# aleju/cat-generator

Measured on AMD Instinct MI355X. Metric: images/sec per G+D step, G32up-c 32x32 RGB bs=128 per GPU, higher is better.
Workload: dtype f32

## Files before the change

cat-generator_amd/csrc/common.h:

```cpp
#pragma once
#include <hip/hip_runtime.h>
#include <algorithm>
#include <stdint.h>
#include <stdio.h>
#include <string.h>
#include "../../include/catgan.h"

namespace cg {

char* err_buf();
int fail(const char* fmt, ...);

inline hipStream_t S(void* s) { return reinterpret_cast<hipStream_t>(s); }

#define CG_HIP(call)                                                              \
    do {                                                                          \
        hipError_t e__ = (call);                                                  \
        if (e__ != hipSuccess)                                                    \
            return cg::fail("%s:%d %s -> %s", __FILE__, __LINE__, #call,          \
                            hipGetErrorString(e__));                              \
    } while (0)

#define CG_LAUNCH_CHECK()                                                         \
    do {                                                                          \
        hipError_t e__ = hipGetLastError();                                       \
        if (e__ != hipSuccess)                                                    \
            return cg::fail("%s:%d kernel launch -> %s", __FILE__, __LINE__,      \
                            hipGetErrorString(e__));                              \
    } while (0)

#define CG_REQUIRE(cond, ...)                                                     \
    do {                                                                          \
        if (!(cond)) return cg::fail(__VA_ARGS__);                                \
    } while (0)

constexpr int kNumCU = 256;

#ifndef CG_TIMING_PROBE
#define CG_TIMING_PROBE 0
#endif
#define CG_PROBE_HALF(fam, T) (((CG_TIMING_PROBE) & (fam)) ? ((T) + 1) / 2 : (T))
constexpr int kEwWgsPerCU = 4, kColReduceWgsPerCU = 1;

enum Opt {
    OPT_SKINNY, OPT_GEMM_BK32, OPT_WINO_BK, OPT_NN_TILE, OPT_TN_TILE, OPT_NN_SPLITS, OPT_TN_SPLITS,
    OPT_XCD_SWIZZLE, OPT_NN_GLDS, OPT_TN_GLDS, OPT_WINO_GLDS, OPT_PAD_SKIP, OPT_WINO3, OPT_WINO_DGRAD_FUSE, OPT_WINO_DGRAD_FUSE_LAUNCHES,
    OPT_COUNT
};
long opt(Opt o);
void opt_count(Opt o);

static inline int cdiv(long a, long b) { return (int)((a + b - 1) / b); }

constexpr size_t kColScratchBytes = 8u << 20;
void* col_scratch(hipStream_t stream);
hipStream_t queue_stream(hipStream_t ref, int cls, int slot);
int queue_class(hipStream_t ref, hipStream_t s);
void wgrad_discard_all();

constexpr int kSkinnyWgradBlocks = 512;
bool skinny_ok(int ngroups, int Cin, int Cout, int kH, int kW, int padH, int padW, int ups);
size_t skinny_wgrad_ws_bytes(int Cin, int Cout);
void skinny_valu_forward(hipStream_t st, const float* x, const float* w, const float* bias, float* y, int N, int H, int W, int Cin, int Cout);
void skinny_valu_wgrad(hipStream_t st, const float* x, const float* dy, float* part, float* bias_part, int N, int H, int W, int Cin, int Cout,
                       int blocks, long ppb);
bool skinny_mfma_ok(int Cin, int Cout, int H, int W);
int skinny_mfma_forward(hipStream_t st, const float* x, const float* w, const float* bias, float* y, int N, int H, int W, int Cin, int Cout);
int skinny_mfma_wgrad(hipStream_t st, const float* x, const float* dy, float* part, float* bias_part, int N, int H, int W, int Cin, int Cout,
                      int max_blocks);

bool head_wgrad_ok(int N, int T, int C, int Co);
int head_wgrad(hipStream_t st, const float* x, const float* dy, float* gw, float* gb, int N, int T, int C, int Co, float scale);
bool wino3_geom_ok(int ngroups, int N, int H, int W, int Cin, int Cout, int kH, int kW, int padH, int padW, int ups);
int wino3_note_pack(hipStream_t st, int n, const float* const* w, float* const* wf, float* const* wb, const int* Cout, const int* Cin,
                    const int* kH, const int* kW, const int* wb_map);
int wino3_forward(hipStream_t st, int ngroups, const float* const* x, const float* const* wpk, const float* const* bias, float* const* y,
                  int N, int H, int W);

static inline int ew_grid(long n, int per_block = 256) {
    long b = (n + per_block - 1) / per_block;
    if (b < 1) b = 1;
    const long cap = (long)kNumCU * kEwWgsPerCU;
    if (b > cap) b = cap;
    return (int)b;
}

constexpr int tile_of_row_c(int l) {
    return ((l < 4 || (l >= 12 && l < 16) || (l >= 20 && l < 28)) ? 0 : 16) +
           ((l < 4 || (l >= 12 && l < 16) || (l >= 20 && l < 28)) ? (l < 4 ? l : (l < 16 ? l - 8 : l - 12)) : (l < 12 ? l - 4 : (l < 20 ? l - 8 : l - 16)));
}
__device__ __forceinline__ int tile_of_row(int l) {
    const bool ga = l < 4 || (l >= 12 && l < 16) || (l >= 20 && l < 28);
    const int rank = ga ? (l < 4 ? l : (l < 16 ? l - 8 : l - 12)) : (l < 12 ? l - 4 : (l < 20 ? l - 8 : l - 16));
    return (ga ? 0 : 16) + rank;
}
__device__ __forceinline__ float u01(uint64_t seed, uint64_t ctr) {
    uint64_t z = seed + (ctr + 1) * 0x9E3779B97F4A7C15ull;
    z = (z ^ (z >> 30)) * 0xBF58476D1CE4E5B9ull;
    z = (z ^ (z >> 27)) * 0x94D049BB133111EBull;
    z = z ^ (z >> 31);
    return (float)(z >> 40) * (1.0f / 16777216.0f);
}
__device__ __forceinline__ float wave_sum(float v) {
#pragma unroll
    for (int off = 32; off > 0; off >>= 1) v += __shfl_down(v, off, 64);
    return v;
}
__device__ __forceinline__ double wave_sum(double v) {
#pragma unroll
    for (int off = 32; off > 0; off >>= 1) v += __shfl_down(v, off, 64);
    return v;
}

#ifndef CG_COL_HANDOVER
#define CG_COL_HANDOVER 3
#endif
__device__ __forceinline__ void st_agent(double* p, double v) {
#if CG_COL_HANDOVER == 4
    const unsigned long long old = __hip_atomic_exchange((unsigned long long*)p, (unsigned long long)__double_as_longlong(v),
                                                         __ATOMIC_RELAXED, __HIP_MEMORY_SCOPE_AGENT);
    asm volatile("" ::"v"(old));
#else
    __hip_atomic_store(p, v, __ATOMIC_RELAXED, __HIP_MEMORY_SCOPE_AGENT);
#endif
}
__device__ __forceinline__ double ld_agent(const double* p) {
#if CG_COL_HANDOVER == 4
    unsigned long long zero = 0ull;
    asm volatile("" : "+v"(zero));
    return __longlong_as_double((long long)__hip_atomic_fetch_or((unsigned long long*)const_cast<double*>(p), zero, __ATOMIC_RELAXED,
                                                                 __HIP_MEMORY_SCOPE_AGENT));
#else
    return __hip_atomic_load(const_cast<double*>(p), __ATOMIC_RELAXED, __HIP_MEMORY_SCOPE_AGENT);
#endif
}

__device__ __forceinline__ bool last_block_arrives(unsigned* counter, unsigned total) {
    __shared__ int last_flag;
#if CG_COL_HANDOVER == 0
    __threadfence();
#else
// ... 77 lines not shown
```

cat-generator_amd/csrc/gemm.hip:

```cpp
#include "common.h"
#include <stdlib.h>
#include <algorithm>
#include <mutex>
#include <type_traits>
#include <unordered_map>
#include <vector>

namespace {

typedef float f32x16 __attribute__((ext_vector_type(16)));
typedef unsigned int u32x4 __attribute__((ext_vector_type(4)));

constexpr int BK = 16;
constexpr unsigned OOB = 0x80000000u;
#ifdef CG_TRACE
__device__ unsigned long long* g_trace;
#define CG_STAMP(slot)                                                                                                  \
    do {                                                                                                                \
        if (threadIdx.x == 0 && g_trace) {                                                                              \
            const long wg = blockIdx.x + (long)gridDim.x * (blockIdx.y + (long)gridDim.y * blockIdx.z);                  \
            g_trace[wg * 8 + (slot)] = wall_clock64();                                                                  \
            if ((slot) == 0) {                                                                                          \
                g_trace[wg * 8 + 4] = __builtin_amdgcn_s_getreg((31 << 11) | 4);                       \
                g_trace[wg * 8 + 5] = __builtin_amdgcn_s_getreg((31 << 11) | 20);                     \
// ... 2312 lines not shown
               bool defer, long xgs, long dgs, long gws_, bool gemm_only) {
    CG_REQUIRE(x && dy && gw, "cg_conv2d_wgrad: null pointer");
    const bool strided = xgs != 0;
    CG_REQUIRE(ngroups >= 1 && ngroups <= (strided ? kMaxStridedGroups : MAXG), "cg_conv2d_wgrad: 1..%d groups per launch", strided ? kMaxStridedGroups : MAXG);
    CG_REQUIRE(!strided || (!gb && !defer), "cg_conv2d_wgrad: strided groups carry no bias gradient and are not deferred");
    TNArgs a;
    memset(&a, 0, sizeof(a));
    if (conv_geom(a.g, N, Hp, Wp, Cin, Cout, kH, kW, padH, padW, ups)) return 1;
    const Geom& g = a.g;
    if (!strided && cg::skinny_ok(ngroups, Cin, Cout, kH, kW, padH, padW, ups) && x[0] && dy[0] && gw[0] && (uintptr_t)x[0] % 16 == 0 && ws &&
        ws_bytes >= cg::skinny_wgrad_ws_bytes(Cin, Cout) && (long)N * Hp * Wp < 0x7fffffffL) {
        hipStream_t st = cg::S(stream);
        const long npix = (long)N * Hp * Wp;
        const long ppb = (npix + cg::kSkinnyWgradBlocks - 1) / cg::kSkinnyWgradBlocks;
        int blocks = (int)((npix + ppb - 1) / ppb);
        float* part = (float*)ws;
        float* bpart = part + (size_t)cg::kSkinnyWgradBlocks * 9 * Cin * Cout;
        float* gb0 = gb ? gb[0] : nullptr;
        if (cg::opt(cg::OPT_SKINNY) == 1 && cg::skinny_mfma_ok(Cin, Cout, Hp, Wp)) {
            blocks = cg::skinny_mfma_wgrad(st, x[0], dy[0], part, gb0 ? bpart : nullptr, N, Hp, Wp, Cin, Cout, cg::kSkinnyWgradBlocks / 2);
            if (blocks < 0) return 1;
        }
        else cg::skinny_valu_wgrad(st, x[0], dy[0], part, gb0 ? bpart : nullptr, N, Hp, Wp, Cin, Cout, blocks, ppb);
        CG_LAUNCH_CHECK();
        RedJob job;
        memset(&job, 0, sizeof(job));
        job.part = part; job.bias_part = bpart;
        job.rp.gw0 = gw[0]; job.rp.gb0 = gb0;
        job.Cin = Cin; job.Cout = Cout; job.k = 3; job.KK = 9; job.pad = 1; job.S = blocks; job.P = 1; job.scale = scale;
        job.sstride = 9L * Cin * Cout; job.gstride = 0; job.bsstride = Cout;
        job.wblocks = cg::cdiv(9L * Cin * Cout, 32); job.bblocks = gb0 ? cg::cdiv(Cout, 32) : 0;
        return small_reduce(st, defer, job, 1);
    }
    if (!strided && !gemm_only && ngroups == 1 && !ups && kH == Hp && kW == Wp && padH == 0 && padW == 0 && cg::opt(cg::OPT_PAD_SKIP) > 0 &&
        cg::opt(cg::OPT_TN_GLDS) && cg::head_wgrad_ok(N, kH * kW, Cin, Cout) && x[0] && dy[0] && gw[0] && (uintptr_t)x[0] % 16 == 0 &&
        (uintptr_t)dy[0] % 16 == 0 && (uintptr_t)gw[0] % 4 == 0)
        return cg::head_wgrad(cg::S(stream), x[0], dy[0], gw[0], gb ? gb[0] : nullptr, N, kH * kW, Cin, Cout, scale) != 0;
    TNPlan p = plan_tn(g, ngroups);
    const size_t need = tn_ws_bytes(g, p, ngroups);
    CG_REQUIRE(ws && ws_bytes >= need, "cg_conv2d_wgrad: workspace too small (%zu < %zu)", ws_bytes, need);
    const int nptr = strided ? 1 : ngroups;
    bool veca = Cin % 4 == 0, vecb = Cout % 4 == 0, any_gb = false;
    for (int i = 0; i < nptr; ++i) {
        CG_REQUIRE(x[i] && dy[i] && gw[i], "cg_conv2d_wgrad: null pointer (group %d)", i);
        veca = veca && ((uintptr_t)x[i] % 16 == 0);
        vecb = vecb && ((uintptr_t)dy[i] % 16 == 0);
        any_gb = any_gb || (gb && gb[i]);
    }
    if (strided) { veca = veca && xgs % 4 == 0; vecb = vecb && dgs % 4 == 0; }
    if (p.pm && !(veca && vecb)) p = plan_tn(g, ngroups, false);
    a.xgs = xgs; a.dgs = dgs;
    set4(a.x0, a.x1, a.x2, a.x3, x, nptr);
    set4(a.d0, a.d1, a.d2, a.d3, dy, nptr);
    a.ngroups = ngroups; a.part = (float*)ws; a.pchunk = p.pchunk;
    a.xcd_swizzle = (int)cg::opt(cg::OPT_XCD_SWIZZLE);
    const int ZP = ngroups * g.nphase;
    const long wplane = (long)g.Ktot * g.Cout;
    a.bias_part = any_gb ? (float*)ws + (size_t)p.splits * ZP * wplane : nullptr;
    hipStream_t st = cg::S(stream);
    dim3 grid(cg::cdiv(g.Ktot, p.tc.bm) * cg::cdiv(g.Cout, p.tc.bn), p.splits, ZP);
    if (p.pm && veca && vecb) a.pm_n = g.M / (g.Hg * g.Wg);
    if (a.pm_n || tng_ok(g, p.pchunk, veca, vecb)) {
        if (p.tc.bm == 128 && p.tc.bn == 128) launch_tng<128, 128, 2, 2>(a, grid, st);
        else if (p.tc.bm == 64 && p.tc.bn == 128) launch_tng<64, 128, 2, 2>(a, grid, st);
        else if (p.tc.bm == 128 && p.tc.bn == 64) launch_tng<128, 64, 2, 2>(a, grid, st);
        else if (p.tc.bm == 64 && p.tc.bn == 64) launch_tng<64, 64, 2, 2>(a, grid, st);
        else launch_tng<128, 32, 4, 1>(a, grid, st);
    }
    else if (p.tc.bm == 128 && p.tc.bn == 128) launch_tn<128, 128, 2, 2>(a, grid, st, veca, vecb);
    else if (p.tc.bm == 64 && p.tc.bn == 128) launch_tn<64, 128, 2, 2>(a, grid, st, veca, vecb);
    else if (p.tc.bm == 128 && p.tc.bn == 64) launch_tn<128, 64, 2, 2>(a, grid, st, veca, vecb);
    else if (p.tc.bm == 64 && p.tc.bn == 64) launch_tn<64, 64, 2, 2>(a, grid, st, veca, vecb);
    else launch_tn<128, 32, 4, 1>(a, grid, st, veca, vecb);
    CG_LAUNCH_CHECK();
    if (gemm_only) return 0;
    const int KK = kH * kW;
    int ci_t = KK == 1 ? 64 : 8;
    while (ci_t > 1 && (size_t)KK * ci_t * 33 * sizeof(float) > 60000) ci_t >>= 1;
    const size_t shb = (size_t)KK * ci_t * 33 * sizeof(float);
    dim3 rgrid(cg::cdiv(Cin, ci_t), cg::cdiv(Cout, 32));
    const long relems = (long)KK * Cin * Cout;
    const long sstride = (long)ZP * wplane;
    const int kp = ups ? phase_kp(kH, padH) : 0;
    if (strided && KK == 1 && !ups && !any_gb && Cin % 32 == 0 && Cout % 32 == 0 && g.nphase == 1) {
        hipLaunchKernelGGL(wgrad_reduce_t_kernel, dim3(Cin / 32, Cout / 32, ngroups), dim3(256), 0, st, (const float*)ws, gw[0], gws_, Cin, Cout,
                           p.splits, sstride, (long)g.nphase * wplane, scale);
        CG_LAUNCH_CHECK();
        return 0;
    }
    if ((long)rgrid.x * rgrid.y < cg::kNumCU) {
        RedJob job;
        memset(&job, 0, sizeof(job));
        job.rp.gws = strided ? gws_ : 0;
        set4(job.rp.gw0, job.rp.gw1, job.rp.gw2, job.rp.gw3, gw, nptr);
        set4(job.rp.gb0, job.rp.gb1, job.rp.gb2, job.rp.gb3, gb, nptr);
        job.part = (const float*)ws; job.bias_part = a.bias_part;
        job.Cin = Cin; job.Cout = Cout; job.k = kH; job.KK = KK; job.pad = padH; job.kp = ups ? kp : 0; job.S = p.splits; job.P = g.nphase;
        job.ups = ups ? 1 : 0; job.scale = scale;
        job.sstride = sstride; job.gstride = (long)g.nphase * wplane; job.bsstride = (long)ZP * Cout;
        job.wblocks = cg::cdiv(relems, 32); job.bblocks = any_gb ? cg::cdiv(Cout, 32) : 0;
        if (defer && KK == 1 && !ups && Cin % 32 == 0 && Cout % 32 == 0 && g.nphase == 1) {
            job.tr = 1; job.wblocks = (Cin / 32) * (Cout / 32);
        } else if (!ups && Cout % 4 == 0 && (uintptr_t)ws % 16 == 0 && sstride % 4 == 0 && job.gstride % 4 == 0) {
            job.v4 = 1; job.wblocks = cg::cdiv(relems, 128);
        }
        return small_reduce(st, defer, job, ngroups);
    }
    for (int gi = 0; gi < ngroups; ++gi) {
        const float* pg = (const float*)ws + (long)gi * g.nphase * wplane;
        float* gwi = strided ? gw[0] + (long)gi * gws_ : gw[gi];
        if (ups)
            hipLaunchKernelGGL(wgrad_reduce_kernel<true>, rgrid, dim3(256), shb, st, pg, gwi, Cin, Cout, kH, KK, padH, kp,
                               p.splits, scale, ci_t, sstride);
        else
            hipLaunchKernelGGL(wgrad_reduce_kernel<false>, rgrid, dim3(256), shb, st, pg, gwi, Cin, Cout, kH, KK, padH,
                               0, p.splits, scale, ci_t, sstride);
        CG_LAUNCH_CHECK();
        if (gb && gb[gi]) {
            hipLaunchKernelGGL(bias_part_reduce_kernel, dim3(cg::cdiv(Cout, 32)), dim3(256), 0, st,
                               (const float*)a.bias_part + (long)gi * g.nphase * Cout, gb[gi], p.splits, g.nphase,
                               (long)ZP * Cout, Cout, scale);
            CG_LAUNCH_CHECK();
        }
    }
    return 0;
}

}

int cg_conv2d_wgrad(void* stream, const float* x, const float* dy, float* gw, float* gb, int N, int Hp, int Wp, int Cin,
                    int Cout, int kH, int kW, int padH, int padW, int ups, float scale, void* ws, size_t ws_bytes) {
    CG_REQUIRE(x && dy && gw, "cg_conv2d_wgrad: null pointer");
    return cg_conv2d_wgrad_grouped(stream, 1, &x, &dy, &gw, &gb, N, Hp, Wp, Cin, Cout, kH, kW, padH, padW, ups, scale, ws,
                                   ws_bytes);
}

static int pack_ci_tile(int Cin, int KK) {
    int t = 1;
    while (t * 2 * KK <= 448 && t < Cin) t *= 2;
    return t;
}

int cg_pack_conv_weight(void* stream, const float* w, float* wf, float* wb, int Cout, int Cin, int kH, int kW) {
    CG_REQUIRE(w && (wf || wb), "cg_pack_conv_weight: null pointer");
    CG_REQUIRE(Cout > 0 && Cin > 0 && kH > 0 && kW > 0, "cg_pack_conv_weight: bad dims");
    const int KK = kH * kW;
    hipLaunchKernelGGL(pack_weight_kernel, dim3(cg::cdiv(Cin, 32), cg::cdiv(Cout, 32), KK), dim3(256), 0, cg::S(stream), w,
                       wf, wb, Cout, Cin, KK, 0);
    CG_LAUNCH_CHECK();
    return cg::wino3_note_pack(cg::S(stream), 1, &w, &wf, &wb, &Cout, &Cin, &kH, &kW, nullptr);
}

int cg_pack_conv_weight_map(void* stream, const float* w, float* wf, float* wbT, int Cout, int Cin, int kH, int kW) {
    CG_REQUIRE(w && (wf || wbT), "cg_pack_conv_weight_map: null pointer");
    CG_REQUIRE(Cout > 0 && Cin > 0 && kH > 0 && kW > 0, "cg_pack_conv_weight_map: bad dims");
    const int KK = kH * kW;
    hipLaunchKernelGGL(pack_weight_kernel, dim3(cg::cdiv(Cin, 32), cg::cdiv(Cout, 32), KK), dim3(256), 0, cg::S(stream), w,
                       wf, wbT, Cout, Cin, KK, 1);
    CG_LAUNCH_CHECK();
    return 0;
}

int cg_pack_conv_weight_batch(void* stream, int n, const float* const* w_canonical, float* const* wf, float* const* wb,
                              const int* Cout, const int* Cin, const int* kH, const int* kW, const int* wb_map) {
    CG_REQUIRE(n >= 0 && w_canonical && wf && wb && Cout && Cin && kH && kW, "cg_pack_conv_weight_batch: null pointer");
    for (int i0 = 0; i0 < n; i0 += kPackBatch) {
        PackBatch b;
        memset(&b, 0, sizeof(b));
        b.n = std::min(kPackBatch, n - i0);
        int blocks = 0;
        for (int e = 0; e < b.n; ++e) {
            const int i = i0 + e;
            CG_REQUIRE(w_canonical[i] && (wf[i] || wb[i]) && Cout[i] > 0 && Cin[i] > 0 && kH[i] > 0 && kW[i] > 0,
                       "cg_pack_conv_weight_batch: bad layer %d", i);
            b.w[e] = w_canonical[i]; b.wf[e] = wf[i]; b.wb[e] = wb[i];
            b.Cout[e] = Cout[i]; b.Cin[e] = Cin[i]; b.KK[e] = kH[i] * kW[i];
            if (wb_map && wb_map[i]) b.map_mask |= 1ull << e;
            b.first[e] = blocks;
            blocks += cg::cdiv(Cin[i], 32) * cg::cdiv(Cout[i], 32) * b.KK[e];
        }
        b.first[b.n] = blocks;
        hipLaunchKernelGGL(pack_weight_batch_kernel, dim3(blocks), dim3(256), 0, cg::S(stream), b);
        CG_LAUNCH_CHECK();
    }
    return cg::wino3_note_pack(cg::S(stream), n, w_canonical, wf, wb, Cout, Cin, kH, kW, wb_map);
}

size_t cg_pack_conv_weight_ups2_floats(int Cout, int Cin, int k, int pad) {
    if (Cout <= 0 || Cin <= 0 || k <= 0 || (k & 1) == 0 || pad != (k - 1) / 2) return 0;
    const int kp = phase_kp(k, pad);
    return (size_t)4 * kp * kp * Cin * Cout;
}

int cg_pack_conv_weight_ups2(void* stream, const float* w, float* wf_ph, float* wb_ph, int Cout, int Cin, int k, int pad) {
    CG_REQUIRE(w && (wf_ph || wb_ph), "cg_pack_conv_weight_ups2: null pointer");
    CG_REQUIRE(Cout > 0 && Cin > 0 && k > 0 && (k & 1) == 1 && pad == (k - 1) / 2,
               "cg_pack_conv_weight_ups2: needs an odd kernel with pad=(k-1)/2");
    const int kp = phase_kp(k, pad);
    CG_REQUIRE(k * k <= 448, "cg_pack_conv_weight_ups2: kernel too large (%d taps)", k * k);
    const dim3 fgrid(cg::cdiv(Cin, 32), cg::cdiv(Cout, 32));
    if (k == 3 || k == 5) {
        if (k == 3)
            hipLaunchKernelGGL(pack_weight_ups2_fast_kernel<3>, fgrid, dim3(256), 0, cg::S(stream), w, wf_ph, wb_ph, Cout, Cin);
        else
            hipLaunchKernelGGL(pack_weight_ups2_fast_kernel<5>, fgrid, dim3(256), 0, cg::S(stream), w, wf_ph, wb_ph, Cout, Cin);
        CG_LAUNCH_CHECK();
        return 0;
    }
    const int ci_t = pack_ci_tile(Cin, k * k);
    hipLaunchKernelGGL(pack_weight_ups2_kernel, dim3(cg::cdiv(Cin, ci_t), cg::cdiv(Cout, 32)), dim3(256),
                       (size_t)32 * (ci_t * k * k + 1) * sizeof(float), cg::S(stream), w, wf_ph, wb_ph, Cout, Cin, k, pad, kp,
                       ci_t);
    CG_LAUNCH_CHECK();
    return 0;
}

}

void cg::wgrad_discard_all() {
    std::lock_guard<std::mutex> lk(g_red_mu);
    for (auto& kv : g_red_queue) kv.second.clear();
}
```

cat-generator_amd/csrc/ops.hip:

```cpp
#include "common.h"
#include <stdarg.h>
#include <stdlib.h>
#include <algorithm>

namespace cg {
char* err_buf() {
    static thread_local char buf[512] = {0};
    return buf;
}
int fail(const char* fmt, ...) {
    va_list ap;
    va_start(ap, fmt);
    vsnprintf(err_buf(), 512, fmt, ap);
    va_end(ap);
    return 1;
}

namespace {
struct OptDef { const char* name; long dflt; };
const OptDef kOptDefs[OPT_COUNT] = {
    {"CG_SKINNY", 1}, {"CG_GEMM_BK32", 1}, {"CG_WINO_BK", 0}, {"CG_NN_TILE", 0}, {"CG_TN_TILE", 0}, {"CG_NN_SPLITS", 0}, {"CG_TN_SPLITS", 0},
    {"CG_XCD_SWIZZLE", 7}, {"CG_NN_GLDS", 1}, {"CG_TN_GLDS", 1}, {"CG_WINO_GLDS", 1}, {"CG_PAD_SKIP", 20}, {"CG_WINO3", 1},
    {"CG_WINO_DGRAD_FUSE", 1}, {"CG_WINO_DGRAD_FUSE_LAUNCHES", 0},
};
long g_opt_val[OPT_COUNT];
int g_opt_state[OPT_COUNT];
}

}
#include <chrono>
#include <mutex>
#include <unordered_map>
#include <vector>
namespace cg {
void* col_scratch(hipStream_t stream) {
    constexpr int kPool = 8, kReserve = 4;
    static std::unordered_map<hipStream_t, void*> blocks;
    static std::vector<void*> pool;
    static std::mutex mu;
    std::lock_guard<std::mutex> lk(mu);
    auto it = blocks.find(stream);
    if (it != blocks.end()) return it->second;
    hipStreamCaptureStatus st = hipStreamCaptureStatusNone;
    const bool capturing = stream && hipStreamIsCapturing(stream, &st) == hipSuccess && st != hipStreamCaptureStatusNone;
    if (capturing && pool.empty()) {
        cg::fail("column reduce: no scratch block left for a stream first used inside a graph capture (run one pass on it before cg_graph_begin)");
        return nullptr;
    }
    if (!capturing && (int)pool.size() <= kReserve) {
        char* p = nullptr;
        hipStreamCaptureMode mode = hipStreamCaptureModeRelaxed;
        (void)hipThreadExchangeStreamCaptureMode(&mode);
        const bool ok = hipMalloc((void**)&p, kColScratchBytes * kPool) == hipSuccess &&
                        hipMemsetAsync(p, 0, kColScratchBytes * kPool, stream) == hipSuccess &&
                        hipStreamSynchronize(stream) == hipSuccess;
        (void)hipThreadExchangeStreamCaptureMode(&mode);
        if (!ok) {
            (void)hipGetLastError();
            if (pool.empty()) { cg::fail("column reduce: cannot allocate %zu bytes of scratch", kColScratchBytes * kPool); return nullptr; }
        } else
            for (int i = kPool - 1; i >= 0; --i) pool.insert(pool.begin(), p + (size_t)i * kColScratchBytes);
    }
    void* blk = pool.back();
    pool.pop_back();
    blocks[stream] = blk;
    return blk;
}
namespace {
__global__ void queue_probe_spin_k(unsigned long long ticks, int* sink) {
    const unsigned long long t0 = wall_clock64();
    while (wall_clock64() - t0 < ticks) { }
    if (ticks == ~0ull) *sink = 1;
}
struct QueuePool {
    std::vector<hipStream_t> s;
    std::unordered_map<hipStream_t, std::vector<int>> cls;
    std::mutex mu;
};
QueuePool& qpool() { static QueuePool p; return p; }
constexpr int kQueuePool = 24;

double probe_pair(hipStream_t a, hipStream_t b, bool both, unsigned long long ticks) {
    (void)hipStreamSynchronize(a);
    if (both) (void)hipStreamSynchronize(b);
    const auto t0 = std::chrono::steady_clock::now();
    hipLaunchKernelGGL(queue_probe_spin_k, dim3(1), dim3(64), 0, a, ticks, (int*)nullptr);
    if (both) hipLaunchKernelGGL(queue_probe_spin_k, dim3(1), dim3(64), 0, b, ticks, (int*)nullptr);
    (void)hipStreamSynchronize(a);
    if (both) (void)hipStreamSynchronize(b);
    return std::chrono::duration<double, std::milli>(std::chrono::steady_clock::now() - t0).count();
}
bool same_queue(hipStream_t a, hipStream_t b) {
    const unsigned long long ticks = 30000;
    int votes = 0;
    for (int r = 0; r < 3; ++r) {
        const double one = probe_pair(a, a, false, ticks), two = probe_pair(a, b, true, ticks);
        if (two > 1.6 * one) ++votes;
    }
    return votes >= 2;
}
}

int queue_classify(hipStream_t ref) {
    QueuePool& p = qpool();
    hipStreamCaptureStatus st = hipStreamCaptureStatusNone;
    if (ref && hipStreamIsCapturing(ref, &st) == hipSuccess && st != hipStreamCaptureStatusNone)
// ... 1863 lines not shown
```

cat-generator_amd/csrc/winograd.hip:

```cpp
#include "common.h"
#include <algorithm>
#include <type_traits>
#include <stdlib.h>

namespace {

typedef float f32x16 __attribute__((ext_vector_type(16)));

__device__ __forceinline__ float4 ld4(const float* p) { return *reinterpret_cast<const float4*>(p); }
__device__ __forceinline__ float wf4c(const float4& v, int i) { return i == 0 ? v.x : (i == 1 ? v.y : (i == 2 ? v.z : v.w)); }
__device__ __forceinline__ float4 f4add(float4 a, float4 b) { return make_float4(a.x + b.x, a.y + b.y, a.z + b.z, a.w + b.w); }
__device__ __forceinline__ float4 f4sub(float4 a, float4 b) { return make_float4(a.x - b.x, a.y - b.y, a.z - b.z, a.w - b.w); }

template <int MODE>
__global__ __launch_bounds__(256) void wino_input_transform_kernel(const float* __restrict__ src, float* __restrict__ V,
                                                                   int N, int Hl, int Wl, int C, int Cs) {
    const int cq_n = C >> 2;
    const int tH = Hl >> 1, tW = Wl >> 1;
    const long T = (long)N * tH * tW;
    const long total = T * cq_n;
    for (long idx = blockIdx.x * 256L + threadIdx.x; idx < total; idx += gridDim.x * 256L) {
        const int cq = (int)(idx % cq_n);
        const long tile = idx / cq_n;
        const int tj = (int)(tile % tW);
// ... 733 lines not shown
#pragma unroll
            for (int o = 0; o < 4; ++o) {
                if (cyr[o >> 1] == 0.f) continue;
#pragma unroll
                for (int ni = 0; ni < 2; ++ni) {
                    f32x16 Y;
                    add_row(o, ni, Y);
                    if (row == 3) store_out(o, ni, Y);
                    else {
                        float* Xo = X + (o * 2 + ni) * 1024;
#pragma unroll
                        for (int r = 0; r < 16; ++r) Xo[r * 64 + lane] = Y[r];
                    }
                }
            }
        } else if (row == 3 && xy < 2) {
#pragma unroll
            for (int ni = 0; ni < 2; ++ni) {
                f32x16 Y;
                const float* Xo = X + (xy * 2 + ni) * 1024;
#pragma unroll
                for (int r = 0; r < 16; ++r) Y[r] = Xo[r * 64 + lane];
                if (xy == 0) store_out(0, ni, Y); else store_out(1, ni, Y);
            }
        }
        if (row < 3) __syncthreads();
    }
}

__global__ __launch_bounds__(256) void wino_dy_transform_kernel(const float* __restrict__ dy, float* __restrict__ Mdy, int N,
                                                                int Hl, int Wl, int Cout, float* __restrict__ bpart) {
    const int C = 4 * Cout, cq_n = C >> 2;
    float4 bacc = make_float4(0.f, 0.f, 0.f, 0.f);
    const int tH = Hl >> 1, tW = Wl >> 1;
    const long T = (long)N * tH * tW;
    const long total = T * cq_n;
    for (long idx = blockIdx.x * 256L + threadIdx.x; idx < total; idx += gridDim.x * 256L) {
        const int cq = (int)(idx % cq_n);
        const long tile = idx / cq_n;
        const int tj = (int)(tile % tW);
        const int ti = (int)((tile / tW) % tH);
        const long n = tile / ((long)tW * tH);
        const int p = (cq * 4) / Cout, co = cq * 4 - p * Cout;
        const int pa = p >> 1, pb = p & 1;
        float4 e[2][2];
#pragma unroll
        for (int u = 0; u < 2; ++u)
#pragma unroll
            for (int v = 0; v < 2; ++v)
                e[u][v] = ld4(dy + ((n * 2 * Hl + 2 * (2 * ti + u) + pa) * (long)(2 * Wl) + 2 * (2 * tj + v) + pb) * Cout + co);
        bacc = f4add(bacc, f4add(f4add(e[0][0], e[0][1]), f4add(e[1][0], e[1][1])));
        float4 r[4][2];
#pragma unroll
        for (int v = 0; v < 2; ++v) {
            r[0][v] = e[0][v];
            r[1][v] = f4add(e[0][v], e[1][v]);
            r[2][v] = f4sub(e[0][v], e[1][v]);
            r[3][v] = make_float4(-e[1][v].x, -e[1][v].y, -e[1][v].z, -e[1][v].w);
        }
        float* out = Mdy + tile * C + cq * 4;
        const long xs = T * C;
#pragma unroll
        for (int xy = 0; xy < 4; ++xy) {
            *reinterpret_cast<float4*>(out + (xy * 4 + 0) * xs) = r[xy][0];
            *reinterpret_cast<float4*>(out + (xy * 4 + 1) * xs) = f4add(r[xy][0], r[xy][1]);
            *reinterpret_cast<float4*>(out + (xy * 4 + 2) * xs) = f4sub(r[xy][0], r[xy][1]);
            *reinterpret_cast<float4*>(out + (xy * 4 + 3) * xs) = make_float4(-r[xy][1].x, -r[xy][1].y, -r[xy][1].z, -r[xy][1].w);
        }
    }
    if (bpart) {
        __shared__ float4 shb[256];
        shb[threadIdx.x] = bacc;
        __syncthreads();
        const int cq = (int)((blockIdx.x * 256L + threadIdx.x) % cq_n);
        if (cq_n >= 256) *reinterpret_cast<float4*>(bpart + (long)blockIdx.x * C + cq * 4) = bacc;
        else if ((int)threadIdx.x < cq_n) {
            float4 t = shb[threadIdx.x];
            for (int j = threadIdx.x + cq_n; j < 256; j += cq_n) t = f4add(t, shb[j]);
            *reinterpret_cast<float4*>(bpart + (long)blockIdx.x * C + cq * 4) = t;
        }
    }
}

__global__ __launch_bounds__(256) void wino_bias_finish_kernel(const float* __restrict__ bpart, int nblocks, int Cout, float* __restrict__ gb,
                                                               float scale) {
    __shared__ double sh[8][33];
    const int cl = threadIdx.x & 31, rl = threadIdx.x >> 5;
    const int co = blockIdx.x * 32 + cl;
    double a = 0.0;
    if (co < Cout)
        for (int b = rl; b < nblocks; b += 8) {
            const float* row = bpart + (long)b * 4 * Cout + co;
            a += ((double)row[0] + (double)row[Cout]) + ((double)row[2 * Cout] + (double)row[3 * Cout]);
        }
    sh[rl][cl] = a;
    __syncthreads();
    if (rl == 0 && co < Cout) {
        double t = 0.0;
#pragma unroll
        for (int r = 0; r < 8; ++r) t += sh[r][cl];
        gb[co] += scale * (float)t;
    }
}

__device__ __host__ __forceinline__ int wino_phase_map(int a, int d) { return ((a + d - 2) >> 1) - ((a - 2) >> 1); }

__global__ __launch_bounds__(256) void wino_wgrad_finish_kernel(const float* __restrict__ dUt, float* __restrict__ gw, int Cout,
                                                                int Cin, float scale) {
    const long total = (long)Cout * Cin;
    const long xs = 4L * Cout * Cin;
    for (long idx = blockIdx.x * 256L + threadIdx.x; idx < total; idx += gridDim.x * 256L) {
        const int ci = (int)(idx % Cin);
        const int co = (int)(idx / Cin);
        float acc[25];
#pragma unroll
        for (int t = 0; t < 25; ++t) acc[t] = 0.f;
#pragma unroll
        for (int p = 0; p < 4; ++p) {
            float u[4][4];
#pragma unroll
            for (int xi = 0; xi < 16; ++xi) u[xi >> 2][xi & 3] = dUt[xi * xs + ((long)p * Cout + co) * Cin + ci];
            float t[3][4];
#pragma unroll
            for (int c = 0; c < 4; ++c) {
                t[0][c] = u[0][c] + 0.5f * (u[1][c] + u[2][c]);
                t[1][c] = 0.5f * (u[1][c] - u[2][c]);
                t[2][c] = 0.5f * (u[1][c] + u[2][c]) + u[3][c];
            }
            float g[3][3];
#pragma unroll
            for (int r = 0; r < 3; ++r) {
                g[r][0] = t[r][0] + 0.5f * (t[r][1] + t[r][2]);
                g[r][1] = 0.5f * (t[r][1] - t[r][2]);
                g[r][2] = 0.5f * (t[r][1] + t[r][2]) + t[r][3];
            }
#pragma unroll
            for (int dy = 0; dy < 5; ++dy)
#pragma unroll
                for (int dx = 0; dx < 5; ++dx) acc[dy * 5 + dx] += g[wino_phase_map(p >> 1, dy)][wino_phase_map(p & 1, dx)];
        }
        float* dst = gw + idx * 25;
#pragma unroll
        for (int t = 0; t < 25; ++t) dst[t] += scale * acc[t];
    }
}


__device__ __host__ __forceinline__ int wino22_phase_map(int a, int d) { return ((a + d - 1) >> 1) - ((a - 1) >> 1); }


static bool wino_dims_ok(int N, int Hp, int Wp, int Cin, int Cout) {
    return N > 0 && Hp > 0 && Wp > 0 && (Hp & 1) == 0 && (Wp & 1) == 0 && Cin > 0 && Cout > 0 && Cin % 128 == 0 &&
           Cout % 128 == 0  && (long)N * Hp * Wp * std::max(Cin, 4 * Cout) * 4L < (1L << 40);
}

}

extern "C" {

size_t cg_conv2d_ups2_wino_supported(int N, int Hp, int Wp, int Cin, int Cout, int k, int pad) {
    return k == 5 && pad == 2 && wino_dims_ok(N, Hp, Wp, Cin, Cout) ? 1 : 0;
}
size_t cg_conv2d_ups2_wino_v_floats(int N, int Hp, int Wp, int C) {
    return (size_t)16 * ((size_t)N * (Hp / 2) * (Wp / 2)) * C;
}
size_t cg_conv2d_ups2_wino_u_floats(int Cin, int Cout) { return (size_t)4 * 16 * Cin * Cout; }
// ... 163 lines not shown
    const long n = (long)T * 4 * Cin;
    if (sl == 4) hipLaunchKernelGGL(wino22_sum_kernel<4>, dim3(cg::ew_grid(n / 4)), dim3(256), 0, cg::S(stream), part, dx_lo, n / 4, n);
    else hipLaunchKernelGGL(wino22_sum_kernel<2>, dim3(cg::ew_grid(n / 4)), dim3(256), 0, cg::S(stream), part, dx_lo, n / 4, n);
    CG_LAUNCH_CHECK();
    return 0;
}

static bool wino_dgrad_fused_takes(const float* dy, const float* u_bwd, const float* dx_lo, int N, int Hp, int Wp, int Cin, int Cout) {
    const long mode = cg::opt(cg::OPT_WINO_DGRAD_FUSE);
    if (mode == 0) return false;
    const int tH = Hp / 2, tW = Wp / 2, bH = cg::cdiv(tH, 8), bW = cg::cdiv(tW, 8);
    const long wgs = (long)N * bH * bW * (Cin / 64);
    const bool fits = 4L * Hp * Wp * Cout * 4L < 0x7fffffffL && (long)Hp * Wp * Cin * 4L < 0x7fffffffL && 16L * 4L * Cout * Cin * 4L < 0x7fffffffL &&
                      Cout % 32 == 0 && Cin % 64 == 0 && wgs <= 0x7fffffffL &&
                      ((uintptr_t)dy % 16) == 0 && ((uintptr_t)u_bwd % 16) == 0 && ((uintptr_t)dx_lo % 4) == 0;
    if (!fits) return false;
    return mode == 2 || (tH % 8 == 0 && tW % 8 == 0 && wgs >= cg::kNumCU);
}

int cg_conv2d_ups2_wino_dgrad(void* stream, const float* dy, const float* u_bwd, float* dx_lo, float* v_dy, int N, int Hp,
                              int Wp, int Cin, int Cout) {
    CG_REQUIRE(dy && u_bwd && dx_lo && v_dy, "cg_conv2d_ups2_wino_dgrad: null pointer");
    CG_REQUIRE(wino_dims_ok(N, Hp, Wp, Cin, Cout), "cg_conv2d_ups2_wino_dgrad: unsupported dimensions");
    hipStream_t st = cg::S(stream);
    if (wino_dgrad_fused_takes(dy, u_bwd, dx_lo, N, Hp, Wp, Cin, Cout)) {
        WinoFusedArgs f;
        f.dy = dy; f.U = u_bwd; f.y = dx_lo; f.N = N; f.tH = Hp / 2; f.tW = Wp / 2; f.Cs = Cout; f.K = 4 * Cout; f.Nc = Cin;
        f.bH = cg::cdiv(f.tH, 8); f.bW = cg::cdiv(f.tW, 8);
        f.xcd = (int)cg::opt(cg::OPT_XCD_SWIZZLE);
        hipLaunchKernelGGL(wino_dgrad_fused_kernel, dim3((unsigned)(N * f.bH * f.bW * (Cin / 64))), dim3(512), 0, st, f);
        CG_LAUNCH_CHECK();
        cg::opt_count(cg::OPT_WINO_DGRAD_FUSE_LAUNCHES);
        return 0;
    }
    const int T = N * (Hp / 2) * (Wp / 2);
    hipLaunchKernelGGL(wino_input_transform_kernel<1>, dim3(cg::ew_grid((long)T * Cout)), dim3(256), 0, st, dy, v_dy, N, Hp, Wp,
                       4 * Cout, Cout);
    CG_LAUNCH_CHECK();
    return cg_conv2d_ups2_wino_gemm(stream, v_dy, u_bwd, nullptr, dx_lo, N, Hp, Wp, Cin, Cout, 1);
}

static int wino_dgrad_slices(int N, int Hp, int Wp, int Cin, int Cout) {
    const int force = 0;
    const long T = (long)N * (Hp / 2) * (Wp / 2);
    const bool glds = cg::opt(cg::OPT_WINO_GLDS) != 0 && T * 4L * Cout * 4L < 0x7fffffffL &&
                      16L * 4L * Cout * Cin * 4L < 0x7fffffffL;
    if (!glds || !wino_dims_ok(N, Hp, Wp, Cin, Cout)) return 1;
    const long wgs = (long)cg::cdiv((int)T, 64) * (Cin / 128);
    int sl = force == 1 || force == 2 || force == 4 ? force : (wgs >= cg::kNumCU ? 1 : (wgs * 2 >= cg::kNumCU ? 2 : 4));
    while (sl > 1 && (4 * Cout / sl) % 64 != 0) sl >>= 1;
    return sl;
}
size_t cg_conv2d_ups2_wino_dgrad_part_floats(int N, int Hp, int Wp, int Cin, int Cout) {
    const int sl = wino_dgrad_slices(N, Hp, Wp, Cin, Cout);
    return sl > 1 ? (size_t)sl * N * Hp * Wp * Cin : 0;
}
int cg_conv2d_ups2_wino_dgrad_split(void* stream, const float* dy, const float* u_bwd, float* dx_lo, float* v_dy, float* part, int N, int Hp,
                                    int Wp, int Cin, int Cout) {
    const int sl = wino_dgrad_slices(N, Hp, Wp, Cin, Cout);
    if (sl <= 1 || !part) return cg_conv2d_ups2_wino_dgrad(stream, dy, u_bwd, dx_lo, v_dy, N, Hp, Wp, Cin, Cout);
    CG_REQUIRE(dy && u_bwd && dx_lo && v_dy, "cg_conv2d_ups2_wino_dgrad_split: null pointer");
    const int T = N * (Hp / 2) * (Wp / 2);
    hipLaunchKernelGGL(wino_input_transform_kernel<1>, dim3(cg::ew_grid((long)T * Cout)), dim3(256), 0, cg::S(stream), dy, v_dy, N, Hp, Wp, 4 * Cout, Cout);
    CG_LAUNCH_CHECK();
    if (wino_gemm_launch(stream, v_dy, u_bwd, nullptr, part, N, Hp, Wp, Cin, Cout, 1, nullptr, 16, sl)) return 1;
    const long n = (long)T * 4 * Cin;
    if (sl == 4) hipLaunchKernelGGL(wino22_sum_kernel<4>, dim3(cg::ew_grid(n / 4)), dim3(256), 0, cg::S(stream), part, dx_lo, n / 4, n);
    else hipLaunchKernelGGL(wino22_sum_kernel<2>, dim3(cg::ew_grid(n / 4)), dim3(256), 0, cg::S(stream), part, dx_lo, n / 4, n);
    CG_LAUNCH_CHECK();
    return 0;
}

static size_t wino_align(size_t b) { return (b + 255) / 256 * 256; }

size_t cg_conv2d_ups2_wino_wgrad_workspace_bytes(int N, int Hp, int Wp, int Cin, int Cout) {
    if (!wino_dims_ok(N, Hp, Wp, Cin, Cout)) return 0;
    const size_t T = (size_t)N * (Hp / 2) * (Wp / 2);
    return wino_align(16 * T * 4 * Cout * sizeof(float)) + wino_align((size_t)16 * 4 * Cout * Cin * sizeof(float)) +
           wino_align(std::max(sizeof(double) * Cout, (size_t)cg::kNumCU * 8 * 4 * Cout * sizeof(float))) +

           cg_conv2d_wgrad_workspace_bytes_strided(16, (int)T, 1, 1, Cin, 4 * Cout, 1, 1, 0, 0, 0);
}

int cg_conv2d_ups2_wino_wgrad(void* stream, const float* v, const float* dy, float* gw_canonical, float* gb, int N, int Hp,
                              int Wp, int Cin, int Cout, float scale, void* ws, size_t ws_bytes) {
    CG_REQUIRE(v && dy && gw_canonical, "cg_conv2d_ups2_wino_wgrad: null pointer");
    CG_REQUIRE(wino_dims_ok(N, Hp, Wp, Cin, Cout), "cg_conv2d_ups2_wino_wgrad: unsupported dimensions");
    const size_t need = cg_conv2d_ups2_wino_wgrad_workspace_bytes(N, Hp, Wp, Cin, Cout);
    CG_REQUIRE(ws && ws_bytes >= need && (uintptr_t)ws % 16 == 0, "cg_conv2d_ups2_wino_wgrad: workspace too small (%zu < %zu)",
               ws_bytes, need);
    hipStream_t st = cg::S(stream);
    const int T = N * (Hp / 2) * (Wp / 2);
    const int C4 = 4 * Cout;
    char* base = (char*)ws;
    float* mdy = (float*)base;                    base += wino_align((size_t)16 * T * C4 * sizeof(float));
    float* dut = (float*)base;                    base += wino_align((size_t)16 * C4 * Cin * sizeof(float));
    const size_t bws_bytes = wino_align(std::max(sizeof(double) * Cout, (size_t)cg::kNumCU * 8 * 4 * Cout * sizeof(float)));
    void* bws = base;                             base += bws_bytes;
    void* tws = base;
    const size_t tws_bytes = ws_bytes - (size_t)(base - (char*)ws);
    const bool fuse = false;
    const int tgrid = (int)cg::ew_grid((long)T * Cout);
    hipLaunchKernelGGL(wino_dy_transform_kernel, dim3(tgrid), dim3(256), 0, st, dy, mdy, N, Hp, Wp, Cout, fuse ? (float*)bws : nullptr);
    CG_LAUNCH_CHECK();
    CG_HIP(hipMemsetAsync(dut, 0, (size_t)16 * C4 * Cin * sizeof(float), st));
    const int groups_per_launch = 16;
    for (int q = 0; q < 16; q += groups_per_launch) {
        if (cg_conv2d_wgrad_strided(stream, groups_per_launch, v + q * (long)T * Cin, (long)T * Cin, mdy + q * (long)T * C4, (long)T * C4,
                                    dut + q * (long)C4 * Cin, (long)C4 * Cin, T, 1, 1, Cin, C4, 1, 1, 0, 0, 0, 1.f, tws, tws_bytes)) return 1;
    }
    hipLaunchKernelGGL(wino_wgrad_finish_kernel, dim3(cg::ew_grid((long)Cout * Cin)), dim3(256), 0, st, dut, gw_canonical, Cout,
                       Cin, scale);
    CG_LAUNCH_CHECK();
    if (fuse) {
        hipLaunchKernelGGL(wino_bias_finish_kernel, dim3(cg::cdiv(Cout, 32)), dim3(256), 0, st, (const float*)bws, tgrid, Cout, gb, scale);
        CG_LAUNCH_CHECK();
        return 0;
    }
    if (gb) return cg_bias_grad(stream, dy, gb, (long)N * 4 * Hp * Wp, Cout, scale, bws, wino_align(sizeof(double) * Cout));
    return 0;
}



}
```

Baseline: 23180.

## Fuse Winograd dy transform into the wgrad GEMM prologue

```diff
diff --git a/cat-generator_amd/csrc/common.h b/cat-generator_amd/csrc/common.h
--- a/cat-generator_amd/csrc/common.h
+++ b/cat-generator_amd/csrc/common.h
@@ -45,7 +45,7 @@
 enum Opt {
     OPT_SKINNY, OPT_GEMM_BK32, OPT_WINO_BK, OPT_NN_TILE, OPT_TN_TILE, OPT_NN_SPLITS, OPT_TN_SPLITS,
     OPT_XCD_SWIZZLE, OPT_NN_GLDS, OPT_TN_GLDS, OPT_WINO_GLDS, OPT_PAD_SKIP, OPT_WINO3, OPT_WINO_DGRAD_FUSE, OPT_WINO_DGRAD_FUSE_LAUNCHES,
-    OPT_COUNT
+    OPT_WINO_WGRAD_FUSE, OPT_WINO_WGRAD_FUSE_LAUNCHES, OPT_COUNT
 };
 long opt(Opt o);
 void opt_count(Opt o);
@@ -57,6 +57,8 @@
 hipStream_t queue_stream(hipStream_t ref, int cls, int slot);
 int queue_class(hipStream_t ref, hipStream_t s);
 void wgrad_discard_all();
+int wgrad_strided_plan(int ngroups, int M, int Cin, int Cout, int* splits, int* pchunk);
+int wgrad_strided_reduce(hipStream_t st, int ngroups, const float* part, float* gw, long gws, int Cin, int Cout, int splits, float scale);
 
 constexpr int kSkinnyWgradBlocks = 512;
 bool skinny_ok(int ngroups, int Cin, int Cout, int kH, int kW, int padH, int padW, int ups);
diff --git a/cat-generator_amd/csrc/gemm.hip b/cat-generator_amd/csrc/gemm.hip
--- a/cat-generator_amd/csrc/gemm.hip
+++ b/cat-generator_amd/csrc/gemm.hip
@@ -2418,12 +2418,8 @@
     const long relems = (long)KK * Cin * Cout;
     const long sstride = (long)ZP * wplane;
     const int kp = ups ? phase_kp(kH, padH) : 0;
-    if (strided && KK == 1 && !ups && !any_gb && Cin % 32 == 0 && Cout % 32 == 0 && g.nphase == 1) {
-        hipLaunchKernelGGL(wgrad_reduce_t_kernel, dim3(Cin / 32, Cout / 32, ngroups), dim3(256), 0, st, (const float*)ws, gw[0], gws_, Cin, Cout,
-                           p.splits, sstride, (long)g.nphase * wplane, scale);
-        CG_LAUNCH_CHECK();
-        return 0;
-    }
+    if (strided && KK == 1 && !ups && !any_gb && Cin % 32 == 0 && Cout % 32 == 0 && g.nphase == 1)
+        return cg::wgrad_strided_reduce(st, ngroups, (const float*)ws, gw[0], gws_, Cin, Cout, p.splits, scale);
     if ((long)rgrid.x * rgrid.y < cg::kNumCU) {
         RedJob job;
         memset(&job, 0, sizeof(job));
@@ -2553,6 +2549,23 @@
 
 }
 
+int cg::wgrad_strided_plan(int ngroups, int M, int Cin, int Cout, int* splits, int* pchunk) {
+    Geom g;
+    if (ngroups < 1 || ngroups > kMaxStridedGroups || conv_geom(g, M, 1, 1, Cin, Cout, 1, 1, 0, 0, 0)) return 1;
+    const TNPlan p = plan_tn(g, ngroups);
+    if (p.pm || !tng_flat(g) || Cin % 32 || Cout % 32) return 1;
+    *splits = p.splits;
+    *pchunk = p.pchunk;
+    return 0;
+}
+int cg::wgrad_strided_reduce(hipStream_t st, int ngroups, const float* part, float* gw, long gws, int Cin, int Cout, int splits, float scale) {
+    const long wplane = (long)Cin * Cout;
+    hipLaunchKernelGGL(wgrad_reduce_t_kernel, dim3(Cin / 32, Cout / 32, ngroups), dim3(256), 0, st, part, gw, gws, Cin, Cout, splits,
+                       (long)ngroups * wplane, wplane, scale);
+    CG_LAUNCH_CHECK();
+    return 0;
+}
+
 void cg::wgrad_discard_all() {
     std::lock_guard<std::mutex> lk(g_red_mu);
     for (auto& kv : g_red_queue) kv.second.clear();
diff --git a/cat-generator_amd/csrc/ops.hip b/cat-generator_amd/csrc/ops.hip
--- a/cat-generator_amd/csrc/ops.hip
+++ b/cat-generator_amd/csrc/ops.hip
@@ -22,6 +22,7 @@
     {"CG_SKINNY", 1}, {"CG_GEMM_BK32", 1}, {"CG_WINO_BK", 0}, {"CG_NN_TILE", 0}, {"CG_TN_TILE", 0}, {"CG_NN_SPLITS", 0}, {"CG_TN_SPLITS", 0},
     {"CG_XCD_SWIZZLE", 7}, {"CG_NN_GLDS", 1}, {"CG_TN_GLDS", 1}, {"CG_WINO_GLDS", 1}, {"CG_PAD_SKIP", 20}, {"CG_WINO3", 1},
     {"CG_WINO_DGRAD_FUSE", 1}, {"CG_WINO_DGRAD_FUSE_LAUNCHES", 0},
+    {"CG_WINO_WGRAD_FUSE", 1}, {"CG_WINO_WGRAD_FUSE_LAUNCHES", 0},
 };
 long g_opt_val[OPT_COUNT];
 int g_opt_state[OPT_COUNT];
diff --git a/cat-generator_amd/csrc/winograd.hip b/cat-generator_amd/csrc/winograd.hip
--- a/cat-generator_amd/csrc/winograd.hip
+++ b/cat-generator_amd/csrc/winograd.hip
@@ -839,6 +839,160 @@
     }
 }
 
+struct WinoWgradFusedArgs {
+    const float* V;
+    const float* dy;
+    float* part;
+    int T, tH, tW, Cin, Cout;
+    int pchunk;
+};
+constexpr int kWgBK = 16;
+
+__device__ __forceinline__ float4 wino_bufld4(__amdgpu_buffer_rsrc_t r, unsigned voff) {
+    typedef unsigned u32x4 __attribute__((ext_vector_type(4)));
+    typedef float f32x4 __attribute__((ext_vector_type(4)));
+    const u32x4 v = __builtin_amdgcn_raw_buffer_load_b128(r, voff, 0, 0);
+    const f32x4 f = __builtin_bit_cast(f32x4, v);
+    return make_float4(f.x, f.y, f.z, f.w);
+}
+
+__global__ __launch_bounds__(256, 2) void wino_wgrad_fused_kernel(WinoWgradFusedArgs a) {
+    constexpr int kHalf = kWgBK * 128;
+    __shared__ __attribute__((aligned(16))) float S0[2 * kHalf];
+    __shared__ __attribute__((aligned(16))) float S1[2 * kHalf];
+    const int tid = threadIdx.x, lane = tid & 63, wave = __builtin_amdgcn_readfirstlane(tid >> 6);
+    const int l31 = lane & 31, h = lane >> 5;
+    const int wm0 = (wave >> 1) * 64, wn0 = (wave & 1) * 64;
+    const int C4 = 4 * a.Cout;
+    const int split = blockIdx.x, xi = blockIdx.z, xy = xi >> 2, xx = xi & 3;
+    const int ntn = C4 >> 7;
+    const int tn = (int)blockIdx.y % ntn, tm = (int)blockIdx.y / ntn;
+    const int m0 = tm * 128, n0 = tn * 128;
+    const int ps = split * a.pchunk, pend = min(a.T, ps + a.pchunk);
+    const int nt = CG_PROBE_HALF(2, (pend - ps + kWgBK - 1) / kWgBK);
+
+    const __amdgpu_buffer_rsrc_t rsv = __builtin_amdgcn_make_buffer_rsrc((void*)a.V, 0, (unsigned)(16 * a.T * a.Cin) * 4u, 0x00020000);
+    unsigned vvoff[2];
+#pragma unroll
+    for (int i = 0; i < 2; ++i) vvoff[i] = (unsigned)(((xi * a.T + 4 * wave + 2 * i + h) * a.Cin + m0 + 4 * l31) * 4);
+    auto dma_v = [&](auto bufc, int p0) {
+        constexpr int buf = decltype(bufc)::value;
+#pragma unroll
+        for (int i = 0; i < 2; ++i)
+            wino_glds16(rsv, (buf ? S1 : S0) + (4 * wave + 2 * i) * 128, p0 + 4 * wave + 2 * i + h < pend ? vvoff[i] : 0x80000000u, p0 * a.Cin * 4);
+    };
+    const __amdgpu_buffer_rsrc_t rsd =
+        __builtin_amdgcn_make_buffer_rsrc((void*)a.dy, 0, (unsigned)(16 * a.T * a.Cout) * 4u, 0x00020000);
+    const int d_kr = tid >> 5, d_q = tid & 31;
+    const int d_col = n0 + 4 * d_q, d_p = d_col / a.Cout, d_co = d_col - d_p * a.Cout;
+    const int W2 = 4 * a.tW;
+    const int d_base = ((d_p >> 1) * W2 + (d_p & 1)) * a.Cout + d_co;
+    const int d_us = 2 * W2 * a.Cout, d_vs = 2 * a.Cout;
+    const bool need_u[2] = {xy != 3, xy != 0}, need_v[2] = {xx != 3, xx != 0};
+    float4 e[2][2][2];
+    auto ld_dy = [&](int p0) {
+#pragma unroll
+        for (int q = 0; q < 2; ++q) {
+            const int tile = p0 + d_kr + 8 * q;
+            const bool ok = tile < pend;
+            const int tc = ok ? tile : 0;
+            const int tj = tc % a.tW, tr = tc / a.tW;
+            const unsigned o = (unsigned)(((tr * 4) * W2 + 4 * tj) * a.Cout + d_base) * 4u;
+#pragma unroll
+            for (int u = 0; u < 2; ++u)
+#pragma unroll
+                for (int v = 0; v < 2; ++v)
+                    e[q][u][v] = wino_bufld4(rsd, ok && need_u[u] && need_v[v] ? o + (unsigned)(u * d_us + v * d_vs) * 4u : 0x80000000u);
+        }
+    };
+    auto st_b = [&](auto bufc) {
+        constexpr int buf = decltype(bufc)::value;
+#pragma unroll
+        for (int q = 0; q < 2; ++q) {
+            float4 r[2];
+#pragma unroll
+            for (int v = 0; v < 2; ++v) {
+                if (xy == 0) r[v] = e[q][0][v];
+                else if (xy == 1) r[v] = f4add(e[q][0][v], e[q][1][v]);
+                else if (xy == 2) r[v] = f4sub(e[q][0][v], e[q][1][v]);
+                else r[v] = make_float4(-e[q][1][v].x, -e[q][1][v].y, -e[q][1][v].z, -e[q][1][v].w);
+            }
+            float4 o;
+            if (xx == 0) o = r[0];
+            else if (xx == 1) o = f4add(r[0], r[1]);
+            else if (xx == 2) o = f4sub(r[0], r[1]);
+            else o = make_float4(-r[1].x, -r[1].y, -r[1].z, -r[1].w);
+            *reinterpret_cast<float4*>((buf ? S1 : S0) + kHalf + (d_kr + 8 * q) * 128 + 4 * d_q) = o;
+        }
+    };
+
+    f32x16 acc[2][2];
+#pragma unroll
+    for (int i = 0; i < 2; ++i)
+#pragma unroll
+        for (int j = 0; j < 2; ++j)
+#pragma unroll
+            for (int r = 0; r < 16; ++r) acc[i][j][r] = 0.f;
+
+    using B0c = std::integral_constant<int, 0>;
+    using B1c = std::integral_constant<int, 1>;
+    if (nt > 0) {
+        dma_v(B0c{}, ps);
+        ld_dy(ps);
+        st_b(B0c{});
+    }
+    asm volatile("s_waitcnt vmcnt(0)" ::: "memory");
+    __syncthreads();
+
+    auto k_tile = [&](auto bufc, int t) {
+        constexpr int buf = decltype(bufc)::value;
+        const bool more = t + 1 < nt;
+        if (more) {
+            dma_v(std::integral_constant<int, buf ^ 1>{}, ps + (t + 1) * kWgBK);
+            ld_dy(ps + (t + 1) * kWgBK);
+        }
+        const float* A = (buf ? S1 : S0) + wm0 + l31;
+        const float* B = (buf ? S1 : S0) + kHalf + wn0 + l31;
+        const unsigned b_addr = (unsigned)(uintptr_t)(__attribute__((address_space(3))) const float*)B + (unsigned)h * 512u;
+        auto k_pair = [&](auto kc) {
+            constexpr int kk = decltype(kc)::value;
+            float av[2], bv[2];
+#pragma unroll
+            for (int i = 0; i < 2; ++i) av[i] = A[(kk + h) * 128 + i * 32];
+            asm volatile("ds_read_b32 %0, %2 offset:%3\n\tds_read_b32 %1, %2 offset:%4\n\ts_waitcnt lgkmcnt(0)"
+                         : "=&v"(bv[0]), "=&v"(bv[1]) : "v"(b_addr), "n"(kk * 512), "n"(kk * 512 + 128) : "memory");
+#pragma unroll
+            for (int i = 0; i < 2; ++i)
+#pragma unroll
+                for (int j = 0; j < 2; ++j) acc[i][j] = __builtin_amdgcn_mfma_f32_32x32x2f32(av[i], bv[j], acc[i][j], 0, 0, 0);
+        };
+        k_pair(std::integral_constant<int, 0>{}); k_pair(std::integral_constant<int, 2>{}); k_pair(std::integral_constant<int, 4>{});
+        k_pair(std::integral_constant<int, 6>{}); k_pair(std::integral_constant<int, 8>{}); k_pair(std::integral_constant<int, 10>{});
+        k_pair(std::integral_constant<int, 12>{}); k_pair(std::integral_constant<int, 14>{});
+        static_assert(kWgBK == 16, "eight k pairs per K step");
+        __builtin_amdgcn_sched_barrier(0);
+        if (more) st_b(std::integral_constant<int, buf ^ 1>{});
+        asm volatile("s_waitcnt vmcnt(0)" ::: "memory");
+        __syncthreads();
+    };
+    for (int t = 0; t < nt; t += 2) {
+        k_tile(B0c{}, t);
+        if (t + 1 < nt) k_tile(B1c{}, t + 1);
+    }
+
+    float* pout = a.part + ((long)split * 16 + xi) * a.Cin * C4;
+    const __amdgpu_buffer_rsrc_t rp = __builtin_amdgcn_make_buffer_rsrc((void*)pout, 0, (unsigned)(a.Cin * C4) * 4u, 0x00020000);
+    const unsigned vo = ((unsigned)(m0 + wm0 + 4 * h) * (unsigned)C4 + (unsigned)(n0 + wn0 + l31)) * 4u;
+#pragma unroll
+    for (int i = 0; i < 2; ++i)
+#pragma unroll
+        for (int r = 0; r < 16; ++r) {
+            const int soff = (i * 32 + (r & 3) + 8 * (r >> 2)) * C4 * 4;
+#pragma unroll
+            for (int j = 0; j < 2; ++j) __builtin_amdgcn_raw_buffer_store_b32(__float_as_uint(acc[i][j][r]), rp, (int)(vo + j * 128), soff, 0);
+        }
+}
+
 __global__ __launch_bounds__(256) void wino_bias_finish_kernel(const float* __restrict__ bpart, int nblocks, int Cout, float* __restrict__ gb,
                                                                float scale) {
     __shared__ double sh[8][33];
@@ -1168,6 +1322,18 @@
            cg_conv2d_wgrad_workspace_bytes_strided(16, (int)T, 1, 1, Cin, 4 * Cout, 1, 1, 0, 0, 0);
 }
 
+static bool wino_wgrad_fused_takes(const float* v, const float* dy, int N, int Hp, int Wp, int Cin, int Cout, int* splits, int* pchunk) {
+    const long mode = cg::opt(cg::OPT_WINO_WGRAD_FUSE);
+    if (mode == 0) return false;
+    const long T = (long)N * (Hp / 2) * (Wp / 2), C4 = 4L * Cout;
+    const bool fits = 16L * T * Cin * 4L < 0x7fffffffL && 16L * T * Cout * 4L < 0x7fffffffL && (long)Cin * C4 * 4L < 0x7fffffffL &&
+                      Cin % 128 == 0 && Cout % 128 == 0 && (Cin / 128) * (C4 / 128) <= 65535 &&
+                      ((uintptr_t)v % 16) == 0 && ((uintptr_t)dy % 16) == 0;
+    if (!fits || cg::wgrad_strided_plan(16, (int)T, Cin, (int)C4, splits, pchunk) || *pchunk % kWgBK) return false;
+    const long wgs = (long)*splits * (Cin / 128) * (C4 / 128) * 16;
+    return mode == 2 || wgs >= cg::kNumCU;
+}
+
 int cg_conv2d_ups2_wino_wgrad(void* stream, const float* v, const float* dy, float* gw_canonical, float* gb, int N, int Hp,
                               int Wp, int Cin, int Cout, float scale, void* ws, size_t ws_bytes) {
     CG_REQUIRE(v && dy && gw_canonical, "cg_conv2d_ups2_wino_wgrad: null pointer");
@@ -1187,11 +1353,24 @@
     const size_t tws_bytes = ws_bytes - (size_t)(base - (char*)ws);
     const bool fuse = false;
     const int tgrid = (int)cg::ew_grid((long)T * Cout);
-    hipLaunchKernelGGL(wino_dy_transform_kernel, dim3(tgrid), dim3(256), 0, st, dy, mdy, N, Hp, Wp, Cout, fuse ? (float*)bws : nullptr);
-    CG_LAUNCH_CHECK();
+    int fsplits = 0, fpchunk = 0;
+    const bool fused_gemm = wino_wgrad_fused_takes(v, dy, N, Hp, Wp, Cin, Cout, &fsplits, &fpchunk);
+    if (!fused_gemm) {
+        hipLaunchKernelGGL(wino_dy_transform_kernel, dim3(tgrid), dim3(256), 0, st, dy, mdy, N, Hp, Wp, Cout, fuse ? (float*)bws : nullptr);
+        CG_LAUNCH_CHECK();
+    }
     CG_HIP(hipMemsetAsync(dut, 0, (size_t)16 * C4 * Cin * sizeof(float), st));
     const int groups_per_launch = 16;
-    for (int q = 0; q < 16; q += groups_per_launch) {
+    if (fused_gemm) {
+        CG_REQUIRE(tws_bytes >= (size_t)fsplits * 16 * Cin * C4 * sizeof(float), "cg_conv2d_ups2_wino_wgrad: workspace too small for the partial sums");
+        WinoWgradFusedArgs f;
+        f.V = v; f.dy = dy; f.part = (float*)tws; f.T = T; f.tH = Hp / 2; f.tW = Wp / 2; f.Cin = Cin; f.Cout = Cout; f.pchunk = fpchunk;
+        hipLaunchKernelGGL(wino_wgrad_fused_kernel, dim3((unsigned)fsplits, (unsigned)((Cin / 128) * (C4 / 128)), 16), dim3(256), 0, st, f);
+        CG_LAUNCH_CHECK();
+        cg::opt_count(cg::OPT_WINO_WGRAD_FUSE_LAUNCHES);
+        if (cg::wgrad_strided_reduce(st, 16, (const float*)tws, dut, (long)C4 * Cin, Cin, C4, fsplits, 1.f)) return 1;
+    }
+    for (int q = fused_gemm ? 16 : 0; q < 16; q += groups_per_launch) {
         if (cg_conv2d_wgrad_strided(stream, groups_per_launch, v + q * (long)T * Cin, (long)T * Cin, mdy + q * (long)T * C4, (long)T * C4,
                                     dut + q * (long)C4 * Cin, (long)C4 * Cin, T, 1, 1, Cin, C4, 1, 1, 0, 0, 0, 1.f, tws, tws_bytes)) return 1;
     }
```

Result: slower. 22700 (-2.1%).
